# anuragranj/cc

Hardware: AMD Instinct MI355X
Metric: train images/sec (832x256, 5-frame sample, 6-scale CC step) (higher is better)
Workload: dtype f32; 1 GPU; full CC: DispResNet6+PoseNetB6+MaskNet6+Back2Future, all losses; per_gpu_batch=4, global_batch=4, height=256, width=832, scales=6, frames=5, parallelism=dp1, hipgraph=True, trained_nets=all, rccl_ranks=1, dead_occlusion_decoders_elided=False, net_streams=2, pipeline=per_network, grad_chunks=False, deterministic=True

## Files before the change

### cc_amd/csrc/conv.hip

```cpp
#include <stdio.h>
#include <stdlib.h>
#include <stddef.h>
#include <string.h>
#include "cc_common.h"
#include "conv_internal.h"
#include "cc_tools.h"
#include "conv_tail.h"
#include "wino_weights.h"
#include "../../include/ccengine.h"
#include <vector>

namespace {

typedef float f32x16 __attribute__((ext_vector_type(16)));
typedef float f32x4 __attribute__((ext_vector_type(4)));

inline int pick_bm_fwd(int M) {
    static const int no16 = cctools::env_flag("CC_CONV_NO_BM16");
    return M > 64 ? 128 : (M > 32 ? 64 : ((M > 16 || no16) ? 32 : 16));
}

using ccint::BK;
using ccint::BN;
using ccint::MAXGRP;
// ... 600 lines not shown
__device__ __forceinline__ void conv_xcd_blocks(int wmajor, int& bx, int& by, int& bz) {
    bx = (int)blockIdx.x; by = (int)blockIdx.y; bz = (int)blockIdx.z;
    if constexpr (!(CC_XCD_MASK & 1)) return;
    if (wmajor < 0) return;
    if (wmajor) {
        const int gx = (int)gridDim.x, gy = (int)gridDim.y;
        const int w = cc_xcd_order(bx + gx * (by + gy * bz), gx * gy * (int)gridDim.z);
        const int r = w / gx;
        bx = w - r * gx;
        bz = r / gy;
        by = r - bz * gy;
    } else {
        bx = cc_xcd_order(bx, (int)gridDim.x);
    }
}

#ifndef CC_PATCH_LB
#define CC_PATCH_LB 4
#endif
template <int BM, int CK, int TPS, int SPLIT>
__global__ __launch_bounds__(256, CC_PATCH_LB) void k_conv_patch(CP g) {
    int bx, by, bz;
    conv_xcd_blocks(g.wmajor, bx, by, bz);
    conv_patch_body<BM, CK, TPS, SPLIT, 0>(g, bx, by, bz);
}
template <int BM, int TPS, int SPLIT>
__global__ __launch_bounds__(256, CC_PATCH_LB) void k_conv_patch_stk(CP g) {
    int bx, by, bz;
    conv_xcd_blocks(g.wmajor, bx, by, bz);
    conv_patch_body<BM, 8, TPS, SPLIT, 1>(g, bx, by, bz);
}

constexpr int MAXCLS = 12;
struct CPM {
    CP c[MAXCLS];
    int n;
    int bx_end[MAXCLS];
    int wmajor;
};

#if defined(__HIP_DEVICE_COMPILE__) && !defined(CC_HIPEMU)
#define CC_MULTI_DESC(a, k) (*(reinterpret_cast<const CP*>((const char*)__builtin_amdgcn_kernarg_segment_ptr() + offsetof(CPM, c)) + (k)))
#else
#define CC_MULTI_DESC(a, k) ((a).c[k])
#endif
#define CC_MULTI_BODY(BM_, CK_, TPS_, STK_)                                                                                   \
    int bx, by, bz;                                                                                                           \
    conv_xcd_blocks(a.wmajor ? 1 : -1, bx, by, bz);        \
    int k = 0, first = 0, end = a.bx_end[0];                                                                                  \
    _Pragma("unroll") for (int q = 0; q < MAXCLS - 1; q++)                                                                    \
        if (q + 1 < a.n && bx >= a.bx_end[q]) { k = q + 1; first = a.bx_end[q]; end = a.bx_end[q + 1]; }                      \
    const CP& g = CC_MULTI_DESC(a, k);                                                                                        \
    if (bz >= g.nsplit || by * BM_ >= g.Mpad) return;                             \
    bx -= first;                                                                                                              \
    if ((CC_XCD_MASK & 1) && !a.wmajor) bx = cc_xcd_order(bx, end - first);                                                   \
    conv_patch_body<BM_, CK_, TPS_, 2, STK_>(g, bx, by, bz);

template <int BM, int CK, int TPS>
__global__ __launch_bounds__(256, CC_PATCH_LB) void k_conv_patch_multi(CPM a) { CC_MULTI_BODY(BM, CK, TPS, 0) }
template <int BM, int TPS>
__global__ __launch_bounds__(256, CC_PATCH_LB) void k_conv_patch_multi_stk(CPM a) { CC_MULTI_BODY(BM, 8, TPS, 1) }

__global__ __launch_bounds__(256) void k_splitk_epilogue(const float* __restrict__ part, int nsplit, long part_stride,
                                                         const float* __restrict__ bias, const float* __restrict__ res,
                                                         float* __restrict__ y, int M, int OHt, int OWt, int so, int oy0,
                                                         int ox0, int OH, int OW, long y_bs, long res_bs, long total,
// ... 54 lines not shown
    const long r = e - (long)n * per;
    const int m = (int)(r / HWt);
    const int t = (int)(r - (long)m * HWt);
    const int ty = t / c.OWt, tx = t - ty * c.OWt;
    const long po = (((long)n * c.M + m) * c.Hp + ty) * c.Wp + tx;
    float v = 0.f;
    {
        for (int z = 0; z < c.nsplit; z += 8) {
            float p8[8];
#pragma unroll
            for (int u = 0; u < 8; u++) p8[u] = (z + u < c.nsplit) ? c.part[(long)(z + u) * c.part_stride + po] : 0.f;
#pragma unroll
            for (int u = 0; u < 8; u++)
                if (z + u < c.nsplit) v += p8[u];
        }
    }
    const long o = (long)m * c.OH * c.OW + (long)(c.oy0 + c.so * ty) * c.OW + (c.ox0 + c.so * tx);
    if (c.bias) v += c.bias[m];
    c.y[(long)n * c.y_bs + o] = conv_tail(v, c.res != nullptr, c.res ? c.res[(long)n * c.res_bs + o] : 0.f, c.res_mul, c.act, c.act_a, c.act_b,
                                          c.add ? c.add[(long)n * c.add_bs + o] : 0.f);
}

struct ConvPlan {
    bool use_patch;
    int wino;
    ccint::WinoPlan wn;
    int Hp, Wp;
    int tw16;
    int ipt, phi;
    int bm, ck, tps, Mpad, Cpad, PH, PWr, PS, ymin, xmin, tiles_x, tiles_y, nsplit, cps, aligned, shift;
    size_t smem, wp_floats, part_floats;
    int wpad;
    size_t pad_floats;
};

inline long conv_tiles(const GG& g, const ConvPlan& p) { return (long)((g.B + p.ipt - 1) / p.ipt) * p.tiles_x * p.tiles_y; }

inline long conv_blocks(const GG& g, const ConvPlan& p, int mult) { return conv_tiles(g, p) * (p.Mpad / p.bm) * (mult > 1 ? mult : 1); }

inline size_t patch_smem(const ConvPlan& p, int tps) {
    const size_t b = (size_t)(2 * tps * p.ck * p.bm + 2 * p.ck * p.PS) * sizeof(float);
    return (p.bm >= 32 && b < 16384) ? 16384 : b;
}

inline void set_split(ConvPlan& p, const GG& g, int nchunk, long want) {
    p.nsplit = 1; p.cps = nchunk;
    if (want >= 2) {
        p.cps = (int)((nchunk + want - 1) / want);
        p.nsplit = (nchunk + p.cps - 1) / p.cps;
    }
    p.part_floats = p.nsplit > 1 ? (size_t)p.nsplit * g.B * g.M * p.Hp * p.Wp : 0;
}

inline bool wino_geometry(const GG& g) {
    return g.Rt == 3 && g.St == 3 && g.si == 1 && g.so == 1 && g.oy0 == 0 && g.ox0 == 0 && (g.dstep == 1 || g.dstep == -1) &&
           g.dy0 == -g.dstep && g.dx0 == -g.dstep && g.IH == g.OH && g.IW == g.OW && g.OHt == g.OH && g.OWt == g.OW && g.Cin > 0 &&
           (long)g.B * g.Cin * g.IH * g.IW < (1l << 26);
}

inline void adopt_wino(ConvPlan& p, const ccint::WinoPlan& w, const GG& g, int wpad = 0) {
    p.wino = 1;
    p.wn = w;
    p.use_patch = true;
    p.bm = ccwino::WBM; p.ck = ccwino::WCK; p.tps = 1;
    p.Mpad = w.Mpad; p.Cpad = w.Cpad;
    p.nsplit = w.nsplit; p.cps = w.cps;
// ... 96 lines not shown
    const long blocks = conv_blocks(g, p, mult);
    const int nchunk = p.Cpad / p.ck;
    long want = 1;
    if (blocks < cctools::env_int("CC_CONV_SPLIT_BELOW", 384) && nchunk >= 4 && !(g.so != 1 && cctools::env_flag("CC_DBG_NO_PARITY_SPLIT"))) {
        want = (cctools::env_int("CC_CONV_SPLIT_TARGET", 512) + blocks - 1) / blocks;
        if (want > nchunk / cctools::env_int("CC_CONV_MINCHUNKS", 1)) want = nchunk / cctools::env_int("CC_CONV_MINCHUNKS", 1);
        if (want > cctools::env_int("CC_CONV_MAXSPLIT", 32)) want = cctools::env_int("CC_CONV_MAXSPLIT", 32);
    }
    set_split(p, g, nchunk, want);
}

inline void plan_balance(ConvPlan& p, const GG& g, int mult) {
    const long blocks = conv_blocks(g, p, mult);
    const int nchunk = p.Cpad / p.ck;
    if (!(blocks >= 256 && nchunk >= 8 && cctools::env_int("CC_CONV_BALANCE", 1))) return;
    const int T = g.Rt * g.St;
    const double mfma_cyc = (p.bm == 128 ? 3072.0 : p.bm == 64 ? 1536.0 : p.bm == 32 ? 768.0 : 384.0) * (p.tps == 3 ? 1.0 : 1.0 / 3.0);
    const double t_stage = mfma_cyc / 2100.0;
    const double stages = (double)nchunk * ((T + p.tps - 1) / p.tps);
    const double out_bytes = 4.0 * g.B * g.M * g.OHt * g.OWt * (mult > 1 ? mult : 1);
    auto cost = [&](int ns) {
        const double k = (double)((blocks * ns + 255) / 256);
        double t = k * (stages / ns) * t_stage + 2.5;
        if (ns > 1) t += 2.0 * ns * out_bytes / 3.0e6 + 5.0;
        return t;
    };
    int best = 1;
    const int cap = nchunk / 4 < 8 ? nchunk / 4 : 8;
    for (int ns = 2; ns <= cap; ns++)
        if (cost(ns) < cost(best)) best = ns;
    if (best > 1 && cost(best) < 0.01 * cctools::env_int("CC_CONV_BALANCE_PCT", 97) * cost(1)) set_split(p, g, nchunk, best);
}

inline ConvPlan plan_conv(const GG& g, int mult = 1) {
    ConvPlan p = {};
    p.ipt = 1;
    if (wino_geometry(g)) {
        const ccint::WinoPlan w = ccint::wino_plan(g.B, g.Cin, g.IH, g.IW, g.M, mult);
        if (w.ok) adopt_wino(p, w, g);
        if (w.ok || plan_wino_padded(p, g, mult)) return p;
    }
    plan_channel_tile(p, g);
    plan_pixel_tile(p, g);
    plan_patch(p, g);
    plan_split(p, g, mult);
    plan_balance(p, g, mult);
    return p;
}

inline size_t conv_ws_floats(const ConvPlan& p) { return 64 + p.wp_floats + p.part_floats + p.pad_floats; }
template <class F> inline F* ws_image(F* area) { return area + 64; }
inline float* ws_slabs(float* area, size_t image_floats) { return area + 64 + image_floats; }

inline void launch_gg_flat(const GG& g, hipStream_t s) {
    const long Ntot = (long)g.B * g.OHt * g.OWt;
    const int bm = pick_bm(g.M);
    dim3 grid((unsigned)((Ntot + BN - 1) / BN), (unsigned)((g.M + bm - 1) / bm));
    if (bm == 128) hipLaunchKernelGGL(HIP_KERNEL_NAME(k_gather_gemm<128>), grid, dim3(256), 0, s, g);
    else if (bm == 64) hipLaunchKernelGGL(HIP_KERNEL_NAME(k_gather_gemm<64>), grid, dim3(256), 0, s, g);
    else hipLaunchKernelGGL(HIP_KERNEL_NAME(k_gather_gemm<32>), grid, dim3(256), 0, s, g);
}

template <auto KERN, class ARGS>
inline void launch_instance(const ARGS& c, dim3 grid, size_t smem, hipStream_t s) {
    static bool big_lds_enabled = false;
    if (smem > 64 * 1024 && !big_lds_enabled) {
        (void)hipFuncSetAttribute(reinterpret_cast<const void*>(KERN), hipFuncAttributeMaxDynamicSharedMemorySize, 160 * 1024);
        big_lds_enabled = true;
    }
    hipLaunchKernelGGL(KERN, grid, dim3(256), smem, s, c);
}

inline bool stacked(const CPM& a) {
    for (int k = 0; k < a.n; k++)
        if (a.c[k].ipt > 1) return true;
    return false;
}

template <int BM, int CK, int TPS>
// ... 27 lines not shown
template <class ARGS>
inline void dispatch_patch(int bm, int ck, int tps, const ARGS& c, dim3 grid, size_t smem, hipStream_t s) {
    if (tps == 3 && ck == 16) dispatch_bm<16, 3>(bm, c, grid, smem, s);
    else if (tps == 3) dispatch_bm<8, 3>(bm, c, grid, smem, s);
    else if (ck == 16) dispatch_bm<16, 1>(bm, c, grid, smem, s);
    else dispatch_bm<8, 1>(bm, c, grid, smem, s);
}

inline CP make_cp(const GG& g, const ConvPlan& p, const float* zeros, const float* wp, float* part) {
    CP c = {};
    c.x = g.x; c.wp = wp; c.zeros = zeros; c.bias = g.bias; c.res = g.res; c.y = g.y; c.part = part;
    c.B = g.B; c.Cin = g.Cin; c.IH = g.IH; c.IW = g.IW; c.x_bs = g.x_bs;
    c.M = g.M; c.Mpad = p.Mpad; c.Cpad = p.Cpad;
    c.Rt = g.Rt; c.St = g.St; c.si = g.si; c.dstep = g.dstep;
    c.dy_base = g.dy0 - p.ymin; c.dx_base = g.dx0 - p.xmin; c.ymin = p.ymin; c.xmin = p.xmin;
    c.PH = p.PH; c.PWr = p.PWr; c.PS = p.PS; c.tw16 = p.tw16; c.ipt = p.ipt; c.phi = p.phi; c.aligned = p.aligned; c.shift = p.shift;
    c.OHt = g.OHt; c.OWt = g.OWt; c.so = g.so; c.oy0 = g.oy0; c.ox0 = g.ox0; c.OH = g.OH; c.OW = g.OW;
    c.y_bs = g.y_bs; c.res_bs = g.res_bs;
    c.tiles_x = p.tiles_x; c.tiles_y = p.tiles_y;
    c.nsplit = p.nsplit; c.cps = p.cps;
    c.part_stride = (long)g.B * g.M * p.Hp * p.Wp;
    c.act = g.act; c.act_a = g.act_a; c.act_b = g.act_b; c.res_mul = g.res_mul;
    c.add = g.add; c.add_bs = g.add_bs;
#ifndef CC_CONV_WMAJOR
#define CC_CONV_WMAJOR 1
#endif
    c.wmajor = (CC_CONV_WMAJOR && (long)g.M * g.Rt * g.St > (long)g.B * g.IH * g.IW) ? 1 : 0;
    c.vec4 = (g.so == 1) && ((g.OW & 3) == 0) && ((g.ox0 & 3) == 0) && ((((uintptr_t)g.y) & 15) == 0) && ((g.y_bs & 3) == 0) &&
             (!g.res || ((((uintptr_t)g.res) & 15) == 0 && (g.res_bs & 3) == 0)) &&
             (!g.add || ((((uintptr_t)g.add) & 15) == 0 && (g.add_bs & 3) == 0));
    return c;
}

inline EPC fill_epc(const GG& g, const ConvPlan& p, const float* part) {
    const bool empty = g.Cin == 0;
    EPC c = {};
    c.part = empty ? nullptr : part; c.bias = g.bias; c.res = g.res; c.add = g.add; c.y = g.y;
    c.Hp = empty ? g.OHt : p.Hp;
    c.Wp = empty ? g.OWt : p.Wp;
    c.part_stride = (long)g.B * g.M * c.Hp * c.Wp;
    c.nsplit = empty ? 0 : p.nsplit;
    c.OHt = g.OHt; c.OWt = g.OWt; c.oy0 = g.oy0; c.ox0 = g.ox0;
    c.total = (empty || p.nsplit > 1) ? (long)g.B * g.M * g.OHt * g.OWt : 0;
    c.M = g.M; c.so = g.so; c.OH = g.OH; c.OW = g.OW; c.y_bs = g.y_bs; c.res_bs = g.res_bs; c.add_bs = g.add_bs;
    c.act = g.act; c.act_a = g.act_a; c.act_b = g.act_b; c.res_mul = g.res_mul;
    return c;
}

inline void launch_splitk_epilogue(const EPC& c, hipStream_t s) {
    hipLaunchKernelGGL(k_splitk_epilogue, dim3((unsigned)((c.total + 255) / 256)), dim3(256), 0, s, c.part, c.nsplit, c.part_stride, c.bias,
                       c.res, c.y, c.M, c.OHt, c.OWt, c.so, c.oy0, c.ox0, c.OH, c.OW, c.y_bs, c.res_bs, c.total, c.act, c.act_a, c.act_b,
                       c.res_mul, c.add, c.add_bs, c.Hp, c.Wp);
}

inline ccint::WinoGeom wino_geom(const GG& g) {
    ccint::WinoGeom w = {};
    w.B = g.B; w.Cin = g.Cin; w.H = g.IH; w.W = g.IW; w.x_bs = g.x_bs; w.M = g.M; w.y_bs = g.y_bs; w.res_bs = g.res_bs; w.add_bs = g.add_bs;
    w.act = g.act; w.act_a = g.act_a; w.act_b = g.act_b; w.res_mul = g.res_mul;
    return w;
}

inline double wino_gflop(const GG& g, const ConvPlan& p) { return 2e-9 * 16.0 * g.B * p.wn.TY * p.wn.TX * (double)g.M * g.Cin; }

inline int wino_flip(const GG& g) { return g.dstep < 0 ? 1 : 0; }

struct PadTab { ccint::PadJob j[2 * MAXGRP]; int n, B, W, Wp; long row_end[2 * MAXGRP]; };
// ... 51 lines not shown
            pr[k].x = xpad;
        }
        ccint::pad_rows_launch(jobs, nj, g0.B, g0.IW, p.wpad, s);
    }
    wg.W = p.wpad;
    wg.x_bs = (long)g0.Cin * g0.IH * p.wpad;
    if (cctools::env_flag("CC_WINO_TRACE"))
        fprintf(stderr, "wino padded input, %d problems: B%d M%d C%d %dx%d -> pitch %d, nsplit %d dstep %d\n", n, g0.B, g0.M, g0.Cin, g0.IH,
                g0.IW, p.wpad, p.nsplit, g0.dstep);
}

inline int head_kernel_of(const GG& g, ccint::HeadConv& h) {
    static const int off = cctools::env_int("CC_NO_HEAD_KERNELS", 0);
    if (off == 1 || (g.Cin > 4 && g.M > 4) || g.Cin < 1 || g.Rt != 3 || g.St != 3 || g.si != 1 || g.so != 1 || g.oy0 != 0 || g.ox0 != 0) return 0;
    if (g.OHt != g.OH || g.OWt != g.OW || g.OH != g.IH || g.OW != g.IW || g.w_ri != 3 || g.w_sj != 1) return 0;
    if (!((g.dstep == 1 && g.dy0 == -1 && g.dx0 == -1) || (g.dstep == -1 && g.dy0 == 1 && g.dx0 == 1))) return 0;
    if (g.res_mul && !g.res) return 0;
    h = ccint::HeadConv{g.x, g.w, g.bias, g.res, g.res_mul ? g.add : nullptr, g.y, g.B, g.Cin, g.IH, g.IW, g.M, g.x_bs, g.y_bs, g.res_bs,
                        g.add_bs, g.w_sm, g.w_sc, (long)g.w0, g.dstep, g.act, g.act_a, g.act_b, g.res_mul};
    if (g.Cin <= 4 && off != 3 && ccint::head_conv_thinc_vec(h) != 0) return 1;
    if (g.M <= 4 && off != 2 && ccint::head_conv_thinm_ok(h)) return 2;
    return 0;
}

struct ClassForm {
    bool ok;
    bool wino;
    int ref;
    int tps, maxy, maxsplit;
    int nc;
    bool stk;
    bool epi;
    size_t smem;
};

inline int kernel_name(int hk, const GG& g, const ConvPlan& p, const ClassForm* f, char* nm, int cap) {
    const int split = p.nsplit > 1 ? 1 : 0;
    if (hk) return snprintf(nm, cap, hk == 1 ? "k_conv_thinc<%d>" : "k_conv_thinm<%d>", hk == 1 ? g.Cin : g.M);
    if (f && !f->wino && f->nc == 0) return snprintf(nm, cap, "k_splitk_epilogue_multi");
    if (g.Cin == 0) return snprintf(nm, cap, "k_splitk_epilogue");
    if (!p.use_patch) return snprintf(nm, cap, "k_gather_gemm<%d>", pick_bm(g.M));
    if (p.wino) return p.wn.tile ? snprintf(nm, cap, "k_wino_f2x3_s<%d, %d>", p.wn.tile, split) : snprintf(nm, cap, "k_wino_f2x3<%d>", split);
    if (f) return f->stk ? snprintf(nm, cap, "k_conv_patch_multi_stk<%d, %d>", p.bm, f->tps)
                         : snprintf(nm, cap, "k_conv_patch_multi<%d, %d, %d>", p.bm, p.ck, f->tps);
    return p.ipt > 1 ? snprintf(nm, cap, "k_conv_patch_stk<%d, %d, %d>", p.bm, p.tps, split)
                     : snprintf(nm, cap, "k_conv_patch<%d, %d, %d, %d>", p.bm, p.ck, p.tps, split);
}

inline void wino_scope_name(const GG& g, const ConvPlan& p, int nprob, char* nm, int cap) {
    const int nl = kernel_name(0, g, p, nullptr, nm, cap);
    if (cctools::env_flag("CC_TIMING_DETAIL"))
        snprintf(nm + nl, cap - nl, " %dx[B%d M%d C%d %dx%d%s t9 k%d] wg%d", nprob, g.B, g.M, g.Cin, g.OH, g.OW, p.wpad ? "(pad)" : "", p.nsplit,
                 nprob * p.wn.nqb * p.wn.nmb * p.nsplit);
}

inline void launch_gg(const GG& g, float* ws, hipStream_t s, const float* prepacked = nullptr, const float* pre_zeros = nullptr,
                      const ConvPlan* plan = nullptr) {
    ccint::HeadConv h;
    const int hk = head_kernel_of(g, h);
    if (hk) {
        char nm[96];
        const int nl = kernel_name(hk, g, ConvPlan(), nullptr, nm, sizeof nm);
        if (cctools::env_flag("CC_TIMING_DETAIL"))
            snprintf(nm + nl, sizeof nm - nl, " B%d M%d C%d %dx%d t9", g.B, g.M, g.Cin, g.OHt, g.OWt);
        cctiming::Scope tsc(nm, 2e-9 * g.B * g.OHt * g.OWt * (double)g.M * g.Cin * 9, s);
        if (cctools::env_flag("CC_HEAD_TRACE"))
            fprintf(stderr, "head kernel %d: B%d M%d C%d %dx%d dstep %d\n", hk, g.B, g.M, g.Cin, g.OHt, g.OWt, g.dstep);
        if (hk == 1 ? ccint::head_conv_thinc_launch(h, s) : ccint::head_conv_thinm_launch(h, s)) return;
    }
    const ConvPlan p = plan ? *plan : plan_conv(g);
    if (!p.use_patch || ws == nullptr) { launch_gg_flat(g, s); return; }
    float* part = ws_slabs(ws, prepacked ? 0 : p.wp_floats);
    char nm[128];
    if (p.wino) {
        if (!prepacked)
            ccint::wino_weights_launch(g.w, ws_image(ws), g.M, g.Cin, p.Cpad, p.Mpad, g.w_sm, g.w_sc, g.w0, g.w_ri, g.w_sj, wino_flip(g), s);
        ccint::WinoProb pr = {g.x, prepacked ? prepacked : ws_image(ws), g.bias, g.res, g.add, g.y, part};
        ccint::WinoGeom wg = wino_geom(g);
        const ClsIn one = {g, p, nullptr, pr.U, part};
        if (p.wpad) wino_pad_inputs(&one, 1, s, &pr, wg);
        bool ok;
        {
            wino_scope_name(g, p, 1, nm, sizeof nm);
            cctiming::Scope tsc(nm, wino_gflop(g, p), s);
            ok = ccint::wino_launch(wg, p.wn, &pr, 1, s);
        }
        if (!ok) { launch_gg_flat(g, s); return; }
        if (p.nsplit > 1) launch_splitk_epilogue(fill_epc(g, p, part), s);
        return;
    }
    const float* zeros = prepacked ? pre_zeros : ws;
    const float* wp = prepacked ? prepacked : ws_image(ws);
    if (!prepacked)
        hipLaunchKernelGGL(k_repack_w, dim3((unsigned)((p.wp_floats + 255) / 256)), dim3(256), 0, s, g.w, ws_image(ws), ws, g.M, g.Cin,
                           p.Mpad, p.Cpad, g.Rt * g.St, g.St, g.w_sm, g.w_sc, g.w0, g.w_ri, g.w_sj);
    const CP c = make_cp(g, p, zeros, wp, part);
    dim3 grid((unsigned)conv_tiles(g, p), (unsigned)(p.Mpad / p.bm), (unsigned)p.nsplit);
    {
        const int nl = kernel_name(0, g, p, nullptr, nm, sizeof nm);
        if (cctools::env_flag("CC_TIMING_DETAIL"))
            snprintf(nm + nl, sizeof nm - nl, " B%d M%d C%d %dx%d t%d k%d wg%d", g.B, g.M, g.Cin, g.OHt, g.OWt, g.Rt * g.St, p.nsplit,
                     (int)(grid.x * grid.y * grid.z));
        cctiming::Scope tsc(nm, 2e-9 * g.B * g.OHt * g.OWt * (double)g.M * g.Cin * g.Rt * g.St, s);
        dispatch_patch(p.bm, p.ck, p.tps, c, grid, p.smem, s);
    }
    if (p.nsplit > 1) launch_splitk_epilogue(fill_epc(g, p, part), s);
}

inline bool same_problem_shape(const GG& a, const GG& b) {
    return a.B == b.B && a.Cin == b.Cin && a.IH == b.IH && a.IW == b.IW && a.x_bs == b.x_bs && a.M == b.M && a.y_bs == b.y_bs &&
           a.res_bs == b.res_bs && a.add_bs == b.add_bs && a.act == b.act && a.act_a == b.act_a && a.act_b == b.act_b &&
           a.res_mul == b.res_mul && a.dstep == b.dstep;
}

inline ClassForm classes_form(const ClsIn* cs, int n, bool idle_taps) {
    ClassForm f = {};
    f.ref = -1;
    if (n < 1 || n > MAXCLS) return f;
    int nw = 0;
    for (int k = 0; k < n; k++) nw += cs[k].p.wino ? 1 : 0;
    if (nw) {
        if (nw != n) return f;
        const ConvPlan& p = cs[0].p;
        for (int k = 0; k < n; k++) {
            const GG& g = cs[k].g;
            if (!cs[k].wp || !same_problem_shape(g, cs[0].g) || cs[k].p.nsplit != p.nsplit || cs[k].p.cps != p.cps) {
                if (cctools::env_flag("CC_WINO_TRACE"))
                    fprintf(stderr, "wino classes declined: k %d wp %p same %d nsplit %d/%d cps %d/%d\n", k, (const void*)cs[k].wp,
                            (int)same_problem_shape(g, cs[0].g), cs[k].p.nsplit, p.nsplit, cs[k].p.cps, p.cps);
                return f;
            }
            if (p.wpad && (cs[k].p.wpad != p.wpad || cs[k].p.part_floats != p.part_floats || !cs[k].part)) return f;
        }
        f.ok = f.wino = true;
        f.nc = n; f.maxsplit = p.nsplit; f.epi = p.nsplit > 1;
        return f;
    }
    f.tps = 3; f.maxsplit = 1; f.maxy = 1;
    if (cctools::env_int("CC_CONV_IDLE_TAPS", 1)) idle_taps = true;
    for (int k = 0; k < n; k++) {
        const ConvPlan& p = cs[k].p;
        if (cs[k].g.Cin == 0) { f.epi = true; continue; }
        if (f.ref < 0) f.ref = k;
        if (!p.use_patch || p.bm != cs[f.ref].p.bm || p.ck != cs[f.ref].p.ck || !cs[k].wp) return f;
        if (p.tps != 3 && !(idle_taps && cs[k].g.Rt * cs[k].g.St < 3 && patch_smem(p, 3) <= 80 * 1024)) f.tps = 1;
        if (p.nsplit > f.maxsplit) f.maxsplit = p.nsplit;
        if (p.Mpad / p.bm > f.maxy) f.maxy = p.Mpad / p.bm;
        if (p.nsplit > 1) f.epi = true;
        if (p.ipt > 1) f.stk = true;
        f.nc++;
    }
    for (int k = 0; k < n; k++) {
        if (cs[k].g.Cin == 0) continue;
        const size_t sm = patch_smem(cs[k].p, f.tps);
        if (sm > f.smem) f.smem = sm;
    }
    f.ok = f.smem <= 80 * 1024;
    return f;
}

inline bool launch_wino_classes(const ClsIn* cs, int n, hipStream_t s) {
    ccint::WinoProb pr[MAXCLS];
    EPM e = {};
    e.n = n;
    int ebx = 0;
    const ConvPlan& p = cs[0].p;
    for (int k = 0; k < n; k++) {
        const GG& g = cs[k].g;
        pr[k] = ccint::WinoProb{g.x, cs[k].wp, g.bias, g.res, g.add, g.y, cs[k].part};
        e.c[k] = fill_epc(g, p, cs[k].part);
        ebx += (int)((e.c[k].total + 255) / 256);
        e.bx_end[k] = ebx;
    }
    ccint::WinoGeom wg = wino_geom(cs[0].g);
    if (p.wpad) wino_pad_inputs(cs, n, s, pr, wg);
    {
        char nm[128];
        wino_scope_name(cs[0].g, p, n, nm, sizeof nm);
        cctiming::Scope tsc(nm, n * wino_gflop(cs[0].g, p), s);
        if (!ccint::wino_launch(wg, p.wn, pr, n, s)) return false;
    }
    if (p.nsplit > 1) hipLaunchKernelGGL(k_splitk_epilogue_multi, dim3((unsigned)ebx), dim3(256), 0, s, e);
    return true;
}

inline bool launch_classes(const ClsIn* cs, int n, const ClassForm& f, hipStream_t s) {
    if (!f.ok) return false;
    if (f.wino) return launch_wino_classes(cs, n, s);
    CPM a = {};
    EPM e = {};
    e.n = n;
    int bx = 0, ebx = 0, nc = 0;
    double gf = 0, wf = 0, xf = 0;
    for (int k = 0; k < n; k++) {
        const GG& g = cs[k].g;
        const ConvPlan& p = cs[k].p;
        e.c[k] = fill_epc(g, p, cs[k].part);
        ebx += (int)((e.c[k].total + 255) / 256);
        e.bx_end[k] = ebx;
        if (g.Cin == 0) continue;
        a.c[nc] = make_cp(g, p, cs[k].zeros, cs[k].wp, cs[k].part);
        bx += (int)conv_tiles(g, p);
        a.bx_end[nc] = bx;
        nc++;
        gf += 2e-9 * g.B * g.OHt * g.OWt * (double)g.M * g.Cin * g.Rt * g.St;
        wf += (double)g.M * g.Cin * g.Rt * g.St;
        xf += (double)g.B * g.Cin * g.IH * g.IW;
    }
    a.n = nc;
    a.wmajor = (CC_CONV_WMAJOR && wf > xf) ? 1 : 0;
    if (nc > 0) {
        dim3 grid((unsigned)bx, (unsigned)f.maxy, (unsigned)f.maxsplit);
        char nm[224];
        int nl = kernel_name(0, cs[f.ref].g, cs[f.ref].p, &f, nm, sizeof nm);
        if (cctools::env_flag("CC_TIMING_DETAIL")) {
            for (int k = 0; k < n && nl < (int)sizeof nm - 48; k++) {
                const GG& g = cs[k].g;
                if (g.Cin == 0) continue;
                int same = 0, first = 1;
                for (int j = 0; j < n; j++) {
                    const GG& h = cs[j].g;
                    const bool eq = h.Cin == g.Cin && h.M == g.M && h.OHt == g.OHt && h.OWt == g.OWt && h.Rt * h.St == g.Rt * g.St &&
                                    cs[j].p.nsplit == cs[k].p.nsplit;
                    if (eq) { same++; if (j < k) first = 0; }
                }
                if (!first) continue;
                nl += snprintf(nm + nl, sizeof nm - nl, " %dx[B%d M%d C%d %dx%d t%d k%d]", same, g.B, g.M, g.Cin, g.OHt, g.OWt,
                               g.Rt * g.St, cs[k].p.nsplit);
            }
            snprintf(nm + nl, sizeof nm - nl, " wg%d", (int)(grid.x * grid.y * grid.z));
        }
        cctiming::Scope tsc(nm, gf, s);
        dispatch_patch(cs[f.ref].p.bm, cs[f.ref].p.ck, f.tps, a, grid, f.smem, s);
    }
    if (f.epi) hipLaunchKernelGGL(k_splitk_epilogue_multi, dim3((unsigned)ebx), dim3(256), 0, s, e);
    return true;
}

inline bool launch_classes(const ClsIn* cs, int n, hipStream_t s, bool idle_taps = false) {
    return launch_classes(cs, n, classes_form(cs, n, idle_taps), s);
// ... 456 lines not shown
```

### cc_amd/csrc/conv_internal.h

```cpp
#pragma once
#include <stddef.h>
#include <hip/hip_runtime.h>

namespace cctiming {
#ifdef CC_TOOLS
struct Scope {
    hipEvent_t e1 = nullptr;
    hipStream_t s;
    Scope(const char* name, double gflop, hipStream_t st, bool active = true);
    ~Scope();
};
#else
struct Scope { Scope(const char*, double, hipStream_t, bool = true) {} };
#endif
}

namespace ccint {

constexpr int MAXGRP = 4;
constexpr int BN = 128;
constexpr int BK = 16;
inline int pick_bm(int M) { return M > 64 ? 128 : (M > 32 ? 64 : 32); }

struct PadJob { const float* src; float* dst; long bs; int rows_per_image; };
void pad_rows_launch(const PadJob* jobs, int n, int B, int W, int Wp, hipStream_t s);

constexpr int RD_LONGS = 16;
struct RedSink { long* out; int cap; int n; };
int wgrad_reduce_emit(RedSink* sink, const long* desc, int n, hipStream_t s);
int wgrad_reduce_launch(const long* desc, int n, hipStream_t s);

size_t wgrad_thin_ws_floats(int B, int M, int AH, int AW, int Cin, int R, int S, int si);
bool wgrad_thin_launch(const float* a, const float* x, float* gw, float* ws, int B, int M, int AH, int AW, long a_bs, int Cin,
                       int IH, int IW, long x_bs, int R, int S, int si, int pad, long o_sm, long o_sc, int accumulate, hipStream_t s,
                       RedSink* sink = nullptr);

bool wgrad_thin_park(bool on);
bool wgrad_thin_parking();
double wgrad_thin_parked_gflop();
void wgrad_thin_flush(hipStream_t s);

void wgrad_thin_name(int B, int M, int AH, int AW, int Cin, int IH, int IW, int R, int S, int si, int pad, char* out, int cap);


struct WinoGeom {
    int B, Cin, H, W; long x_bs;
    int M; long y_bs, res_bs, add_bs;
    int act; float act_a, act_b; int res_mul;
};
struct WinoProb { const float* x; const float* U; const float* bias; const float* res; const float* add; float* y; float* part; };
struct WinoPlan {
    int ok;
    int Mpad, Cpad, nchunk;
    int TY, TX, nqb, nmb;
    int nsplit, cps;
    int Hp, Wp;
    size_t u_floats, part_floats;
    int tile;
};
constexpr int WINO_MAXP = 12;
WinoPlan wino_plan(int B, int Cin, int H, int W, int M, int mult);
bool wino_launch(const WinoGeom& g, const WinoPlan& p, const WinoProb* probs, int nprob, hipStream_t s);
void wino_weights_launch(const float* w, float* U, int M, int Cin, int Cpad, int Mpad, long w_sm, long w_sc, long w0, long w_ri,
                         long w_sj, int flip, hipStream_t s);

struct WinoWgradPlan {
    int ok;
    int TX, CPR, CPI, NCH;
    int nmb, ncb, Cp;
    int nsplit, cps;
    size_t ws_floats;
};
WinoWgradPlan wino_wgrad_plan(int B, int M, int H, int W, int Cin, int G, int minq = -1);
WinoWgradPlan wino_wgrad_plan_parked(const WinoWgradPlan& alone, int M);
constexpr int WINO_WGRAD_PARK_CAP = 96;
struct WinoWgradParked {
// ... 32 lines not shown
```

Baseline: 249.9 images/s.

## Add persistent M=16 MFMA conv kernel with register-resident weights for thin-output convs

Adds a dedicated kernel for convolutions with at most 16 output channels. It keeps all weights in registers, double-buffers input patches into LDS via global_load_lds, and loops persistently over output tiles. It is routed for large 3x3 stride-1 convs in batched multi-class launches, plus a multi-problem variant that shares the grid in proportion to work. It aims to cut the per-block weight reloads and launch overhead of the generic patch kernel, at the cost of register pressure and heuristic routing that may not beat the existing path.

```diff
diff --git a/cc_amd/csrc/conv.hip b/cc_amd/csrc/conv.hip
--- a/cc_amd/csrc/conv.hip
+++ b/cc_amd/csrc/conv.hip
@@ -656,6 +656,7 @@
 }
 
 constexpr int MAXCLS = 12;
+static_assert(MAXCLS == ccint::M16_MAXCLS, "k_conv_m16_multi takes the class lists of k_conv_patch_multi");
 struct CPM {
     CP c[MAXCLS];
     int n;
@@ -776,6 +777,8 @@
     size_t smem, wp_floats, part_floats;
     int wpad;
     size_t pad_floats;
+    int m16;
+    int m16_tpw;
 };
 
 inline long conv_tiles(const GG& g, const ConvPlan& p) { return (long)((g.B + p.ipt - 1) / p.ipt) * p.tiles_x * p.tiles_y; }
@@ -938,6 +941,28 @@
     if (best > 1 && cost(best) < 0.01 * cctools::env_int("CC_CONV_BALANCE_PCT", 97) * cost(1)) set_split(p, g, nchunk, best);
 }
 
+constexpr int M16_MINPIX = 400000;
+constexpr size_t M16_ROUTED_SMEM = 40 * 1024;
+inline int m16_tiles(const GG& g) { return g.B * ((g.OHt + ccint::M16_TH - 1) / ccint::M16_TH) * ((g.OWt + ccint::M16_TW - 1) / ccint::M16_TW); }
+inline int m16_tpw() {
+    const int forced = cctools::env_int("CC_CONV_M16_TPW", 0);
+    return forced > 0 ? forced : 0;
+}
+inline void plan_m16(ConvPlan& p, const GG& g, int mult) {
+    p.m16 = 0;
+    if (cctools::env_flag("CC_CONV_NO_M16") || !p.use_patch || p.wino || p.bm != 16 || p.ck != 8 || p.Mpad != 16 || p.ipt > 1 ||
+        p.nsplit > 1 || !p.aligned)
+        return;
+    if (g.si != 1 || (g.so != 1 && g.so != 2) || !ccint::m16_grid_ok(g.Rt, g.St, g.dstep, g.Cin)) return;
+    if (!cctools::env_flag("CC_CONV_M16_ALL") &&
+        (mult < 2 || g.so != 1 || g.Rt * g.St != 9 || ccint::m16_smem(g.Rt, g.St, g.Cin) > M16_ROUTED_SMEM))
+        return;
+    if ((long)g.OH * g.OW >= (1l << 26)) return;
+    if ((long)(mult > 1 ? mult : 1) * g.B * g.OHt * g.OWt < cctools::env_int("CC_CONV_M16_MINPIX", M16_MINPIX)) return;
+    p.m16 = 1;
+    p.m16_tpw = m16_tpw();
+}
+
 inline ConvPlan plan_conv(const GG& g, int mult = 1) {
     ConvPlan p = {};
     p.ipt = 1;
@@ -951,6 +976,7 @@
     plan_patch(p, g);
     plan_split(p, g, mult);
     plan_balance(p, g, mult);
+    plan_m16(p, g, mult);
     return p;
 }
 
@@ -1044,6 +1070,20 @@
     return c;
 }
 
+inline ccint::M16Prob make_m16(const GG& g, const ConvPlan& p, const float* zeros, const float* wp) {
+    ccint::M16Prob c = {};
+    c.x = g.x; c.wp = wp; c.zeros = zeros; c.bias = g.bias; c.res = g.res; c.add = g.add; c.y = g.y;
+    c.x_bs = g.x_bs; c.y_bs = g.y_bs; c.res_bs = g.res_bs; c.add_bs = g.add_bs;
+    c.B = g.B; c.Cin = g.Cin; c.IH = g.IH; c.IW = g.IW; c.M = g.M; c.Cpad = p.Cpad;
+    c.Rt = g.Rt; c.St = g.St; c.dstep = g.dstep; c.ymin = p.ymin; c.xmin = p.xmin; c.shift = p.shift;
+    c.OHt = g.OHt; c.OWt = g.OWt; c.so = g.so; c.oy0 = g.oy0; c.ox0 = g.ox0; c.OH = g.OH; c.OW = g.OW;
+    c.tiles_x = (g.OWt + ccint::M16_TW - 1) / ccint::M16_TW;
+    c.tiles_y = (g.OHt + ccint::M16_TH - 1) / ccint::M16_TH;
+    c.ntiles = m16_tiles(g);
+    c.act = g.act; c.act_a = g.act_a; c.act_b = g.act_b; c.res_mul = g.res_mul;
+    return c;
+}
+
 inline EPC fill_epc(const GG& g, const ConvPlan& p, const float* part) {
     const bool empty = g.Cin == 0;
     EPC c = {};
@@ -1161,6 +1201,8 @@
     bool stk;
     bool epi;
     size_t smem;
+    bool m16;
+    int m16_dir, m16_tpw;
 };
 
 inline int kernel_name(int hk, const GG& g, const ConvPlan& p, const ClassForm* f, char* nm, int cap) {
@@ -1170,6 +1212,8 @@
     if (g.Cin == 0) return snprintf(nm, cap, "k_splitk_epilogue");
     if (!p.use_patch) return snprintf(nm, cap, "k_gather_gemm<%d>", pick_bm(g.M));
     if (p.wino) return p.wn.tile ? snprintf(nm, cap, "k_wino_f2x3_s<%d, %d>", p.wn.tile, split) : snprintf(nm, cap, "k_wino_f2x3<%d>", split);
+    if (f && f->m16) return snprintf(nm, cap, "k_conv_m16_multi<%d>", f->m16_dir);
+    if (!f && p.m16 && p.nsplit == 1) return snprintf(nm, cap, "k_conv_m16<%d, %d, %d>", g.Rt, g.St, g.dstep);
     if (f) return f->stk ? snprintf(nm, cap, "k_conv_patch_multi_stk<%d, %d>", p.bm, f->tps)
                          : snprintf(nm, cap, "k_conv_patch_multi<%d, %d, %d>", p.bm, p.ck, f->tps);
     return p.ipt > 1 ? snprintf(nm, cap, "k_conv_patch_stk<%d, %d, %d>", p.bm, p.tps, split)
@@ -1223,6 +1267,15 @@
     if (!prepacked)
         hipLaunchKernelGGL(k_repack_w, dim3((unsigned)((p.wp_floats + 255) / 256)), dim3(256), 0, s, g.w, ws_image(ws), ws, g.M, g.Cin,
                            p.Mpad, p.Cpad, g.Rt * g.St, g.St, g.w_sm, g.w_sc, g.w0, g.w_ri, g.w_sj);
+    if (p.m16 && p.nsplit == 1) {
+        const ccint::M16Prob c = make_m16(g, p, zeros, wp);
+        const int nl = kernel_name(0, g, p, nullptr, nm, sizeof nm);
+        if (cctools::env_flag("CC_TIMING_DETAIL"))
+            snprintf(nm + nl, sizeof nm - nl, " B%d M%d C%d %dx%d t%d tpw%d", g.B, g.M, g.Cin, g.OHt, g.OWt, g.Rt * g.St, p.m16_tpw);
+        cctiming::Scope tsc(nm, 2e-9 * g.B * g.OHt * g.OWt * (double)g.M * g.Cin * g.Rt * g.St, s);
+        ccint::conv_m16_launch(c, p.m16_tpw, s);
+        return;
+    }
     const CP c = make_cp(g, p, zeros, wp, part);
     dim3 grid((unsigned)conv_tiles(g, p), (unsigned)(p.Mpad / p.bm), (unsigned)p.nsplit);
     {
@@ -1266,6 +1319,7 @@
         return f;
     }
     f.tps = 3; f.maxsplit = 1; f.maxy = 1;
+    f.m16 = true;
     if (cctools::env_int("CC_CONV_IDLE_TAPS", 1)) idle_taps = true;
     for (int k = 0; k < n; k++) {
         const ConvPlan& p = cs[k].p;
@@ -1277,7 +1331,16 @@
         if (p.Mpad / p.bm > f.maxy) f.maxy = p.Mpad / p.bm;
         if (p.nsplit > 1) f.epi = true;
         if (p.ipt > 1) f.stk = true;
+        if (!p.m16 || p.nsplit > 1 || cs[k].g.dstep != cs[f.ref].g.dstep) f.m16 = false;
         f.nc++;
+    }
+    if (f.nc == 0) f.m16 = false;
+    if (f.m16) {
+        f.m16_dir = cs[f.ref].g.dstep;
+        f.m16_tpw = m16_tpw();
+        f.stk = false;
+        f.ok = true;
+        return f;
     }
     for (int k = 0; k < n; k++) {
         if (cs[k].g.Cin == 0) continue;
@@ -1335,6 +1398,27 @@
         gf += 2e-9 * g.B * g.OHt * g.OWt * (double)g.M * g.Cin * g.Rt * g.St;
         wf += (double)g.M * g.Cin * g.Rt * g.St;
         xf += (double)g.B * g.Cin * g.IH * g.IW;
+    }
+    if (f.m16) {
+        ccint::M16Table t = {};
+        for (int k = 0; k < n; k++)
+            if (cs[k].g.Cin != 0) t.c[t.n++] = make_m16(cs[k].g, cs[k].p, cs[k].zeros, cs[k].wp);
+        t.tpw = f.m16_tpw;
+        char nm[224];
+        int nl = kernel_name(0, cs[f.ref].g, cs[f.ref].p, &f, nm, sizeof nm);
+        if (cctools::env_flag("CC_TIMING_DETAIL")) {
+            for (int k = 0; k < n && nl < (int)sizeof nm - 48; k++) {
+                const GG& g = cs[k].g;
+                if (g.Cin != 0) nl += snprintf(nm + nl, sizeof nm - nl, " [B%d M%d C%d %dx%d t%d]", g.B, g.M, g.Cin, g.OHt, g.OWt, g.Rt * g.St);
+            }
+            snprintf(nm + nl, sizeof nm - nl, " tpw%d", t.tpw);
+        }
+        {
+            cctiming::Scope tsc(nm, gf, s);
+            if (!ccint::conv_m16_launch_multi(t, s)) return false;
+        }
+        if (f.epi) hipLaunchKernelGGL(k_splitk_epilogue_multi, dim3((unsigned)ebx), dim3(256), 0, s, e);
+        return true;
     }
     a.n = nc;
     a.wmajor = (CC_CONV_WMAJOR && wf > xf) ? 1 : 0;
diff --git a/cc_amd/csrc/conv_internal.h b/cc_amd/csrc/conv_internal.h
--- a/cc_amd/csrc/conv_internal.h
+++ b/cc_amd/csrc/conv_internal.h
@@ -42,6 +42,32 @@
 
 void wgrad_thin_name(int B, int M, int AH, int AW, int Cin, int IH, int IW, int R, int S, int si, int pad, char* out, int cap);
 
+
+constexpr int M16_TH = 4, M16_TW = 32;
+constexpr int M16_MAXCLS = 12;
+constexpr int M16_MAXW = 72;
+constexpr int M16_MAXQ = 18;
+constexpr size_t M16_MAX_SMEM = 80 * 1024;
+__host__ __device__ constexpr int m16_pwr(int St) { return ((M16_TW + St - 1 + 3 + 3) / 4) * 4; }
+__host__ __device__ constexpr int m16_ps(int Rt, int St) { return (((M16_TH + Rt - 1) * m16_pwr(St) - 16 + 31) / 32) * 32 + 16; }
+__host__ __device__ constexpr int m16_qmax(int Rt, int St) { return M16_MAXW / (Rt * St) < M16_MAXQ ? M16_MAXW / (Rt * St) : M16_MAXQ; }
+inline size_t m16_smem(int Rt, int St, int Cin) { return (size_t)2 * ((((Cin + 3) / 4) * 4 * m16_ps(Rt, St) + 255) & ~255) * sizeof(float); }
+inline bool m16_grid_ok(int Rt, int St, int dstep, int Cin) {
+    return Rt >= 1 && Rt <= 3 && St >= 1 && St <= 3 && (dstep == 1 || dstep == -1) && Cin >= 1 && (Cin + 3) / 4 <= m16_qmax(Rt, St) &&
+           m16_smem(Rt, St, Cin) <= M16_MAX_SMEM;
+}
+struct M16Prob {
+    const float* x; const float* wp; const float* zeros; const float* bias; const float* res; const float* add; float* y;
+    long x_bs, y_bs, res_bs, add_bs;
+    int B, Cin, IH, IW, M, Cpad;
+    int Rt, St, dstep, ymin, xmin, shift;
+    int OHt, OWt, so, oy0, ox0, OH, OW;
+    int tiles_x, tiles_y, ntiles;
+    int act; float act_a, act_b; int res_mul;
+};
+struct M16Table { M16Prob c[M16_MAXCLS]; int n; int bx_end[M16_MAXCLS]; int tpw; };
+bool conv_m16_launch(const M16Prob& g, int tpw, hipStream_t s);
+bool conv_m16_launch_multi(M16Table& a, hipStream_t s);
 
 struct WinoGeom {
     int B, Cin, H, W; long x_bs;
diff --git a/cc_amd/csrc/conv_m16.hip b/cc_amd/csrc/conv_m16.hip
--- /dev/null
+++ b/cc_amd/csrc/conv_m16.hip
@@ -0,0 +1,303 @@
+#include <stddef.h>
+#include "cc_common.h"
+#include "conv_internal.h"
+#include "conv_tail.h"
+
+namespace {
+
+using namespace cctail;
+using ccint::M16Prob;
+using ccint::M16Table;
+using ccint::m16_ps;
+using ccint::m16_qmax;
+
+typedef float f32x4 __attribute__((ext_vector_type(4)));
+
+#if defined(CC_HIPEMU)
+#define CC_M16_GLDS16(gsrc, lds_ptr) __builtin_amdgcn_global_load_lds(CC_GLOBAL_PTR(gsrc), CC_LDS_PTR(lds_ptr), 16, 0, 0)
+#else
+__device__ __forceinline__ void m16_glds16(const void* gsrc, unsigned lds_dst) {
+    unsigned keep;
+    asm volatile(
+        "s_mov_b32 %0, m0\n\t"
+        "s_mov_b32 m0, %2\n\t"
+        "s_nop 0\n\t"
+        "global_load_lds_dwordx4 %1, off\n\t"
+        "s_mov_b32 m0, %0"
+        : "=&s"(keep)
+        : "v"(gsrc), "s"(lds_dst)
+        : "memory");
+}
+#define CC_M16_GLDS16(gsrc, lds_ptr) m16_glds16((gsrc), __builtin_amdgcn_readfirstlane((unsigned)(uintptr_t)CC_LDS_PTR(lds_ptr)))
+#endif
+
+template <int RT, int ST, int DIR>
+__device__ __forceinline__ void conv_m16_body(const M16Prob& g, const int t_beg, const int t_end, float* smem) {
+    constexpr int T = RT * ST;
+    constexpr int PH = ccint::M16_TH + RT - 1;
+    constexpr int PWR = ccint::m16_pwr(ST);
+    constexpr int PS = m16_ps(RT, ST);
+    constexpr int QPC = PS / 4, CPR = PWR / 4;
+    constexpr int QMAX = m16_qmax(RT, ST);
+    if (t_beg >= t_end) return;
+
+    const int tid = threadIdx.x, lane = tid & 63;
+    const int wid = __builtin_amdgcn_readfirstlane(tid >> 6);
+    const int l15 = lane & 15, l4 = lane >> 4;
+    const int nq = (g.Cin + 3) >> 2;
+    const int npiece = nq * 4 * QPC;
+    const int bufsz = (nq * 4 * PS + 255) & ~255;
+    const int x_cs = g.IH * g.IW;
+
+    int tx_i = t_beg % g.tiles_x;
+    int ty_i = (t_beg / g.tiles_x) % g.tiles_y;
+    int n = t_beg / (g.tiles_x * g.tiles_y);
+
+    auto load_patch = [&](int n_, int ty_, int tx_, int buf) {
+        float* dst = smem + buf * bufsz;
+        const float* xn = g.x + (long)n_ * g.x_bs;
+        const int gy0 = ty_ * ccint::M16_TH + g.ymin, gx0 = tx_ * ccint::M16_TW + g.xmin - g.shift;
+        for (int q0 = wid * 64; q0 < npiece; q0 += 256) {
+            const int q = q0 + lane;
+            const int c = q / QPC, r = q - c * QPC;
+            const int py = r / CPR, qx = r - py * CPR;
+            const int iy = gy0 + py, ix = gx0 + 4 * qx;
+            const bool ok = q < npiece && py < PH && c < g.Cin && (unsigned)iy < (unsigned)g.IH && (unsigned)ix < (unsigned)g.IW;
+            const float* src = ok ? xn + (long)c * x_cs + (long)iy * g.IW + ix : g.zeros;
+            CC_M16_GLDS16(src, dst + 4 * q0);
+        }
+    };
+
+    const int y_cs = g.OH * g.OW;
+    const bool hr = g.res != nullptr;
+    int buf = 0;
+    load_patch(n, ty_i, tx_i, 0);
+
+    float wr[T][QMAX];
+    {
+        const float* wl = g.wp + l4 * 16 + l15;
+#pragma unroll
+        for (int t = 0; t < T; t++)
+#pragma unroll
+            for (int q = 0; q < QMAX; q++) wr[t][q] = q < nq ? wl[((long)t * g.Cpad + 4 * q) * 16] : 0.f;
+    }
+    const bool hb = g.bias != nullptr;
+    float bv[4];
+#pragma unroll
+    for (int r = 0; r < 4; r++) bv[r] = (hb && 4 * l4 + r < g.M) ? g.bias[4 * l4 + r] : 0.f;
+    CC_WAIT_VMCNT0();
+
+    for (int t = t_beg; t < t_end; t++) {
+        CC_WAIT_VMCNT0_FENCE();
+        __syncthreads();
+        int tx_n = tx_i + 1, ty_n = ty_i, n_n = n;
+        if (tx_n == g.tiles_x) {
+            tx_n = 0;
+            if (++ty_n == g.tiles_y) { ty_n = 0; n_n++; }
+        }
+        if (t + 1 < t_end) load_patch(n_n, ty_n, tx_n, buf ^ 1);
+
+        f32x4 acc0 = {0.f, 0.f, 0.f, 0.f}, acc1 = {0.f, 0.f, 0.f, 0.f};
+        const float* Pl = smem + buf * bufsz + l4 * PS + wid * PWR + l15 + g.shift;
+#pragma unroll
+        for (int ch = 0; ch < QMAX / 2; ch++) {
+            if (2 * ch >= nq) break;
+            if (2 * ch + 1 < nq) {
+#pragma unroll
+                for (int ti = 0; ti < RT; ti++)
+#pragma unroll
+                    for (int tj = 0; tj < ST; tj++) {
+                        const int tapoff = (DIR > 0 ? ti : RT - 1 - ti) * PWR + (DIR > 0 ? tj : ST - 1 - tj);
+#pragma unroll
+                        for (int ks = 0; ks < 2; ks++) {
+                            const float b0 = Pl[(2 * ch + ks) * 4 * PS + tapoff], b1 = Pl[(2 * ch + ks) * 4 * PS + tapoff + 16];
+                            acc0 = __builtin_amdgcn_mfma_f32_16x16x4f32(wr[ti * ST + tj][2 * ch + ks], b0, acc0, 0, 0, 0);
+                            acc1 = __builtin_amdgcn_mfma_f32_16x16x4f32(wr[ti * ST + tj][2 * ch + ks], b1, acc1, 0, 0, 0);
+                        }
+                    }
+            } else {
+#pragma unroll
+                for (int ti = 0; ti < RT; ti++)
+#pragma unroll
+                    for (int tj = 0; tj < ST; tj++) {
+                        const int tapoff = (DIR > 0 ? ti : RT - 1 - ti) * PWR + (DIR > 0 ? tj : ST - 1 - tj);
+                        const float b0 = Pl[(2 * ch) * 4 * PS + tapoff], b1 = Pl[(2 * ch) * 4 * PS + tapoff + 16];
+                        acc0 = __builtin_amdgcn_mfma_f32_16x16x4f32(wr[ti * ST + tj][2 * ch], b0, acc0, 0, 0, 0);
+                        acc1 = __builtin_amdgcn_mfma_f32_16x16x4f32(wr[ti * ST + tj][2 * ch], b1, acc1, 0, 0, 0);
+                    }
+            }
+        }
+
+        const int ty = ty_i * ccint::M16_TH + wid;
+        if (ty < g.OHt) {
+            const int tx = tx_i * ccint::M16_TW + l15;
+            const unsigned vo0 = (unsigned)((g.oy0 + g.so * ty) * g.OW + g.ox0 + g.so * tx + 4 * l4 * y_cs);
+            const unsigned vo[2] = {vo0, vo0 + 16u * (unsigned)g.so};
+            const bool txok[2] = {tx < g.OWt, tx + 16 < g.OWt};
+            float rv[2][4], av[2][4];
+#pragma unroll
+            for (int r = 0; r < 4; r++) {
+                const float* rb = g.res + ((long)n * g.res_bs + (long)r * y_cs);
+                const float* ab = g.add + ((long)n * g.add_bs + (long)r * y_cs);
+#pragma unroll
+                for (int h = 0; h < 2; h++) {
+                    const bool live = txok[h] && 4 * l4 + r < g.M;
+                    rv[h][r] = (hr && live) ? rb[vo[h]] : 0.f;
+                    av[h][r] = (g.add && live) ? ab[vo[h]] : 0.f;
+                }
+            }
+            const int form = (hr && g.res_mul) ? ((g.act == ACT_RELU || g.act == ACT_LRELU) ? 2 : 0) : (g.act != ACT_SIGMOID ? 1 : 0);
+            const float slope = g.act == ACT_LRELU ? (g.act_b != 0.f ? g.act_b : 0.2f) : 1.f;
+#pragma unroll
+            for (int r = 0; r < 4; r++) {
+                float* yb = g.y + ((long)n * g.y_bs + (long)r * y_cs);
+#pragma unroll
+                for (int h = 0; h < 2; h++) {
+                    float v = h ? acc1[r] : acc0[r];
+                    if (hb) v += bv[r];
+                    if (form == 1) {
+                        if (hr) v += rv[h][r];
+                        const float neg = g.act == ACT_RELU ? 0.f : slope * v;
+                        v = (v > 0.f || g.act == ACT_NONE) ? v : neg;
+                    } else if (form == 2) {
+                        const float gsum = v + av[h][r];
+                        const float neg = g.act == ACT_RELU ? 0.f : slope * gsum;
+                        v = rv[h][r] > 0.f ? gsum : neg;
+                    } else {
+                        v = conv_tail(v, hr, rv[h][r], g.res_mul, g.act, g.act_a, g.act_b, av[h][r]);
+                    }
+                    if (txok[h] && 4 * l4 + r < g.M) yb[vo[h]] = v;
+                }
+            }
+        }
+        tx_i = tx_n; ty_i = ty_n; n = n_n;
+        buf ^= 1;
+    }
+}
+
+#ifndef CC_M16_LB
+#define CC_M16_LB 4
+#endif
+
+__device__ __forceinline__ void m16_run(int b, int nwg, int ntiles, int tpw, int& t_beg, int& t_end) {
+    if (tpw > 0) {
+        t_beg = b * tpw;
+        t_end = t_beg + tpw < ntiles ? t_beg + tpw : ntiles;
+    } else {
+        t_beg = (int)((long)b * ntiles / nwg);
+        t_end = (int)((long)(b + 1) * ntiles / nwg);
+    }
+}
+
+template <int RT, int ST, int DIR>
+__global__ __launch_bounds__(256, CC_M16_LB) void k_conv_m16(M16Prob g, int tpw) {
+    HIP_DYNAMIC_SHARED(float, smem)
+    int b = (int)blockIdx.x;
+    if constexpr ((CC_XCD_MASK & 1) != 0) b = cc_xcd_order(b, (int)gridDim.x);
+    int t_beg, t_end;
+    m16_run(b, (int)gridDim.x, g.ntiles, tpw, t_beg, t_end);
+    conv_m16_body<RT, ST, DIR>(g, t_beg, t_end, smem);
+}
+
+#if defined(__HIP_DEVICE_COMPILE__) && !defined(CC_HIPEMU)
+#define CC_M16_DESC(a, k) (*(reinterpret_cast<const M16Prob*>((const char*)__builtin_amdgcn_kernarg_segment_ptr() + offsetof(M16Table, c)) + (k)))
+#else
+#define CC_M16_DESC(a, k) ((a).c[k])
+#endif
+
+template <int DIR>
+__global__ __launch_bounds__(256, CC_M16_LB) void k_conv_m16_multi(M16Table a) {
+    HIP_DYNAMIC_SHARED(float, smem)
+    int b = (int)blockIdx.x;
+    int k = 0, first = 0, end = a.bx_end[0];
+#pragma unroll
+    for (int q = 0; q < ccint::M16_MAXCLS - 1; q++)
+        if (q + 1 < a.n && b >= a.bx_end[q]) { k = q + 1; first = a.bx_end[q]; end = a.bx_end[q + 1]; }
+    const M16Prob& g = CC_M16_DESC(a, k);
+    b -= first;
+    if constexpr ((CC_XCD_MASK & 1) != 0) b = cc_xcd_order(b, end - first);
+    int t_beg, t_end;
+    m16_run(b, end - first, g.ntiles, a.tpw, t_beg, t_end);
+    switch (g.Rt * 4 + g.St) {
+        case 1 * 4 + 1: conv_m16_body<1, 1, DIR>(g, t_beg, t_end, smem); break;
+        case 1 * 4 + 2: conv_m16_body<1, 2, DIR>(g, t_beg, t_end, smem); break;
+        case 1 * 4 + 3: conv_m16_body<1, 3, DIR>(g, t_beg, t_end, smem); break;
+        case 2 * 4 + 1: conv_m16_body<2, 1, DIR>(g, t_beg, t_end, smem); break;
+        case 2 * 4 + 2: conv_m16_body<2, 2, DIR>(g, t_beg, t_end, smem); break;
+        case 2 * 4 + 3: conv_m16_body<2, 3, DIR>(g, t_beg, t_end, smem); break;
+        case 3 * 4 + 1: conv_m16_body<3, 1, DIR>(g, t_beg, t_end, smem); break;
+        case 3 * 4 + 2: conv_m16_body<3, 2, DIR>(g, t_beg, t_end, smem); break;
+        case 3 * 4 + 3: conv_m16_body<3, 3, DIR>(g, t_beg, t_end, smem); break;
+        default: break;
+    }
+}
+
+template <auto KERN, class... ARGS>
+inline void launch_inst(dim3 grid, size_t smem, hipStream_t s, const ARGS&... args) {
+    static bool big_lds_enabled = false;
+    if (smem > 64 * 1024 && !big_lds_enabled) {
+        (void)hipFuncSetAttribute(reinterpret_cast<const void*>(KERN), hipFuncAttributeMaxDynamicSharedMemorySize, 160 * 1024);
+        big_lds_enabled = true;
+    }
+    hipLaunchKernelGGL(KERN, grid, dim3(256), smem, s, args...);
+}
+
+template <int RT, int ST>
+inline void launch_dir(const M16Prob& g, int tpw, dim3 grid, size_t smem, hipStream_t s) {
+    if (g.dstep > 0) launch_inst<&k_conv_m16<RT, ST, 1>>(grid, smem, s, g, tpw);
+    else launch_inst<&k_conv_m16<RT, ST, -1>>(grid, smem, s, g, tpw);
+}
+
+}
+
+inline int m16_slots(size_t smem) {
+    const int per_cu = (int)(160 * 1024 / (smem + 512));
+    return 256 * (per_cu < 1 ? 1 : (per_cu > 4 ? 4 : per_cu));
+}
+
+bool ccint::conv_m16_launch(const M16Prob& g, int tpw, hipStream_t s) {
+    if (!m16_grid_ok(g.Rt, g.St, g.dstep, g.Cin) || tpw < 0 || g.ntiles < 1) return false;
+    const size_t smem = m16_smem(g.Rt, g.St, g.Cin);
+    const int slots = m16_slots(smem);
+    const dim3 grid((unsigned)(tpw > 0 ? (g.ntiles + tpw - 1) / tpw : (g.ntiles < slots ? g.ntiles : slots)));
+    switch (g.Rt * 4 + g.St) {
+        case 1 * 4 + 1: launch_dir<1, 1>(g, tpw, grid, smem, s); break;
+        case 1 * 4 + 2: launch_dir<1, 2>(g, tpw, grid, smem, s); break;
+        case 1 * 4 + 3: launch_dir<1, 3>(g, tpw, grid, smem, s); break;
+        case 2 * 4 + 1: launch_dir<2, 1>(g, tpw, grid, smem, s); break;
+        case 2 * 4 + 2: launch_dir<2, 2>(g, tpw, grid, smem, s); break;
+        case 2 * 4 + 3: launch_dir<2, 3>(g, tpw, grid, smem, s); break;
+        case 3 * 4 + 1: launch_dir<3, 1>(g, tpw, grid, smem, s); break;
+        case 3 * 4 + 2: launch_dir<3, 2>(g, tpw, grid, smem, s); break;
+        default: launch_dir<3, 3>(g, tpw, grid, smem, s); break;
+    }
+    return true;
+}
+
+bool ccint::conv_m16_launch_multi(M16Table& a, hipStream_t s) {
+    if (a.n < 1 || a.n > M16_MAXCLS || a.tpw < 0) return false;
+    size_t smem = 0;
+    double work = 0;
+    for (int k = 0; k < a.n; k++) {
+        const M16Prob& g = a.c[k];
+        if (!m16_grid_ok(g.Rt, g.St, g.dstep, g.Cin) || g.dstep != a.c[0].dstep || g.ntiles < 1) return false;
+        const size_t sm = m16_smem(g.Rt, g.St, g.Cin);
+        if (sm > smem) smem = sm;
+        work += (double)g.ntiles * g.Rt * g.St * ((g.Cin + 3) / 4);
+    }
+    const int slots = m16_slots(smem);
+    int bx = 0;
+    for (int k = 0; k < a.n; k++) {
+        const M16Prob& g = a.c[k];
+        int nwg = (g.ntiles + (a.tpw > 0 ? a.tpw : 1) - 1) / (a.tpw > 0 ? a.tpw : 1);
+        if (a.tpw == 0) {
+            const int share = (int)(slots * ((double)g.ntiles * g.Rt * g.St * ((g.Cin + 3) / 4) / work) + 0.5);
+            nwg = share < 1 ? 1 : (share > g.ntiles ? g.ntiles : share);
+        }
+        bx += nwg;
+        a.bx_end[k] = bx;
+    }
+    if (a.c[0].dstep > 0) launch_inst<&k_conv_m16_multi<1>>(dim3((unsigned)bx), smem, s, a);
+    else launch_inst<&k_conv_m16_multi<-1>>(dim3((unsigned)bx), smem, s, a);
+    return true;
+}
```

New measurement: 250.1 images/s, median of 2. No clear change (+0.1%).
